# BuzzLord/godot-audio-spatializer

Measured on AMD Instinct MI355X. Metric: mixed AudioFrames/s, higher is better.
Workload: dtype f32

## Files before the change

### godot-audio-spatializer_amd/csrc/k_hrtf_multi.hip

```cpp
#define GAS_USE_NT 1
#ifndef GAS_MULTI_L2_PREFETCH
#define GAS_MULTI_L2_PREFETCH 0
#endif
#include "gas_hrtf_wave.h"

namespace {

constexpr int MW = 8;
constexpr int MAXB = GAS_HRTF_MULTI_MAX_BLOCKS;

template <int SQ>
struct MultiLds {
	static constexpr int SLICES_F2 = MW * LDS_F2_HALF;
	static constexpr int FD_F2 = MW * 2 * 512;
	static constexpr int TOTAL_F2 = SLICES_F2 + FD_F2;
	static constexpr int HL = (8 - SQ) * 64;
	static constexpr int LEFT_BYTES = 160 * 1024 - TOTAL_F2 * 8 - 1024 * 8 - 64;
	static constexpr int HIST_ROWS = LEFT_BYTES / (MW * HL * 4);
};

__device__ __forceinline__ void lds_wait_at_least(const uint32_t *flag, uint32_t want) {
	while (__atomic_load_n(flag, __ATOMIC_RELAXED) < want) {
		__builtin_amdgcn_s_sleep(1);
	}
	__builtin_amdgcn_fence(__ATOMIC_ACQUIRE, "workgroup");
}

template <int SQ, bool HIST_LDS>
__global__ __launch_bounds__(MW * 64, GAS_HRTF_WAVES_PER_SIMD) void k_hrtf_multi(gas_group_args g, gas_hrtf_blocks mb, const uint32_t *__restrict__ peak_bits, uint32_t peak_all, gas_dev_state st, gas_hrtf_table tab, const float2 *__restrict__ tw, float *__restrict__ partials) {
	constexpr int FQ = 2 * SQ;
	constexpr int HQ = 8 - SQ;
	constexpr int NQ = 8 + SQ;
	constexpr uint32_t F = FQ * 64;
	constexpr uint32_t HL = HQ * 64;
	__shared__ float2 lds_all[MultiLds<SQ>::TOTAL_F2];
	__shared__ float2 tw_lds[1024];
	__shared__ float hist_lds[HIST_LDS ? MW * MultiLds<SQ>::HIST_ROWS * HL : 4];
	__shared__ uint32_t arrived, consumed;
	const int lane = threadIdx.x & 63;
	const int wave = __builtin_amdgcn_readfirstlane(threadIdx.x >> 6);
	float2 *lds = lds_all + wave * LDS_F2_HALF;
	float *my_hist = hist_lds + (HIST_LDS ? wave * MultiLds<SQ>::HIST_ROWS * HL : 0);
	float2 *fd = lds_all + MultiLds<SQ>::SLICES_F2;
	const uint32_t K = mb.k;

	const float4 tw_in = reinterpret_cast<const float4 *>(tw)[threadIdx.x & 511];
	if (threadIdx.x == 0) {
		arrived = 0;
		consumed = 0;
	}
	uint32_t first, last;
	wave_range(g.n, blockIdx.x * MW + wave, gridDim.x * MW, first, last);
	const uint32_t cnt = last - first;
	const bool have = (uint32_t)lane < cnt;
	uint32_t my_slot = 0, my_row = 0, my_dir = 0, my_flag = 0;
	float my_g0 = 0.0f, my_g1 = 0.0f;
	if (have) {
		const uint32_t e = first + lane;
		my_slot = g.slots ? g.slots[e] : g.slot_base + e;
		my_row = g.rows ? g.rows[e] : e;
	}
	gas_audio_frame raw[FQ];
	float rawh[HQ];
	if (cnt > 0) {
		const uint32_t s0 = (uint32_t)__builtin_amdgcn_readlane((int)my_slot, 0), r0 = (uint32_t)__builtin_amdgcn_readlane((int)my_row, 0);
		load_history<HQ>(st.hrtf_hist + (size_t)s0 * HL, lane, rawh);
#pragma unroll
		for (int q = 0; q < FQ; q++) {
			raw[q] = (GAS_ABL & 8) ? gas_audio_frame{ (float)lane, (float)r0 } : nt_load_frame(mb.src[0] + (size_t)r0 * F + lane + 64 * q);
		}
	}
	auto block_params = [&](uint32_t b, float keep_g, uint32_t keep_d, float &g1, uint32_t &d) {
		const gas_params *fr = mb.fresh[b];
		g1 = keep_g;
		d = keep_d;
		if (have && (fr || b == 0)) {
			const gas_params *P = fr ? fr + my_row : st.params + my_slot;
			const float2 gd = *reinterpret_cast<const float2 *>(&P->hrtf_gain);
			const uint32_t dd = __float_as_uint(gd.y);
			g1 = gd.x;
			d = dd < tab.dirs ? dd : 0;
		}
	};
	if (have) {
		my_g0 = st.hrtf_prev_gain[my_slot];
		const uint32_t e = first + lane;
		my_flag = peak_all ? 1u : (peak_bits ? (peak_bits[e >> 5] >> (e & 31)) & 1u : 0u);
	}
	block_params(0, 0.0f, 0, my_g1, my_dir);
	if (threadIdx.x < 512) {
		reinterpret_cast<float4 *>(tw_lds)[threadIdx.x] = tw_in;
	}
	__syncthreads();
	float2 t1[8], t2[8];
#pragma unroll
	for (int k = 0; k < 8; k++) {
		t1[k] = tw_lds[k * 64 + lane];
		t2[k] = tw_lds[(8 + k) * 64 + lane];
	}
	const float lane_f = (float)lane;
#if GAS_MULTI_L2_PREFETCH
	uint32_t pf_word = 0;
#endif

	for (uint32_t b = 0; b < K; b++) {
		float *peaks_b = mb.peaks[b];
		float2 aYL[8], aYR[8], zp[8];
		float4 hs[8];
#pragma unroll
		for (int j = 0; j < 8; j++) {
			aYL[j] = make_float2(0.0f, 0.0f);
			aYR[j] = make_float2(0.0f, 0.0f);
			zp[j] = make_float2(0.0f, 0.0f);
		}
		float nx_g1 = my_g1;
		uint32_t nx_dir = my_dir;
		if (b + 1 < K) {
			block_params(b + 1, my_g1, my_dir, nx_g1, nx_dir);
		}
		bool have_prev = false;
		uint32_t prev_flag = 0, prev_row = 0;
		auto products = [&](bool more, uint32_t next_dir) {
			float2 yl[8], yr[8];
			if (have_prev) {
				finish_spectra(lane, hs);
#pragma unroll
				for (int j = 0; j < 8; j++) {
					cmac_fixed(aYL[j], zp[j], hs[j].x, hs[j].y);
					cmac_fixed(aYR[j], zp[j], hs[j].z, hs[j].w);
				}
				if (prev_flag) {
#pragma unroll
					for (int j = 0; j < 8; j++) {
						yl[j] = cmul_fixed(zp[j], hs[j].x, hs[j].y);
						yr[j] = cmul_fixed(zp[j], hs[j].z, hs[j].w);
					}
				}
			}
			if (more) {
				issue_spectra(tab.spec, next_dir, lane, hs);
			}
			if (have_prev && prev_flag) {
				fft512<true>(yl, t1, t2, lds, lane);
				fft512<true>(yr, t1, t2, lds, lane);
				float pkl = 0.0f, pkr = 0.0f;
#pragma unroll
				for (int t = 0; t < SQ; t++) {
					pkl = fmaxf(pkl, fmaxf(fabsf(yl[HQ + t].x), fabsf(yl[HQ + t].y)));
					pkr = fmaxf(pkr, fmaxf(fabsf(yr[HQ + t].x), fabsf(yr[HQ + t].y)));
				}
				pkl = wave_max(pkl);
				pkr = wave_max(pkr);
				if (lane == 0) {
					peaks_b[(size_t)prev_row * 2] = pkl;
					peaks_b[(size_t)prev_row * 2 + 1] = pkr;
				}
			}
		};

		for (uint32_t i = 0; i < cnt; i++) {
			const uint32_t slot = (uint32_t)__builtin_amdgcn_readlane((int)my_slot, (int)i);
			const uint32_t row = (uint32_t)__builtin_amdgcn_readlane((int)my_row, (int)i);
			const uint32_t dir = (uint32_t)__builtin_amdgcn_readlane((int)my_dir, (int)i);
			const float g0 = __int_as_float(__builtin_amdgcn_readlane(__float_as_int(my_g0), (int)i));
			const float g1 = __int_as_float(__builtin_amdgcn_readlane(__float_as_int(my_g1), (int)i));
			const uint32_t flag = (uint32_t)__builtin_amdgcn_readlane((int)my_flag, (int)i);
			float xq[NQ];
			if (HIST_LDS && b > 0) {
				load_history<HQ>(my_hist + (size_t)i * HL, lane, rawh);
			}
#pragma unroll
			for (int q = 0; q < HQ; q++) {
				xq[q] = rawh[q];
			}
			float lf = lane_f;
			asm volatile("" : "+v"(lf));
#pragma unroll
			for (int q = 0; q < FQ; q++) {
				const float mono = (raw[q].left + raw[q].right) * 0.5f;
				const float t = (lf + (float)(64 * q)) * (1.0f / (float)F);
				xq[HQ + q] = mono * (g1 * t + (1 - t) * g0);
			}
			if (!HIST_LDS || b + 1 == K) {
				store_history<HQ>(st.hrtf_hist + (size_t)slot * HL, lane, &xq[FQ]);
			} else {
				store_history<HQ>(my_hist + (size_t)i * HL, lane, &xq[FQ]);
			}
			const bool wrap = i + 1 == cnt;
			if (!wrap || b + 1 < K) {
				const uint32_t ni = wrap ? 0u : i + 1;
				const uint32_t nslot = (uint32_t)__builtin_amdgcn_readlane((int)my_slot, (int)ni);
				const uint32_t nrow = (uint32_t)__builtin_amdgcn_readlane((int)my_row, (int)ni);
				const gas_audio_frame *nsrc = mb.src[wrap ? b + 1 : b] + (size_t)nrow * F;
				if (!HIST_LDS || (b == 0 && !wrap)) {
					load_history<HQ>(st.hrtf_hist + (size_t)nslot * HL, lane, rawh);
				}
#pragma unroll
				for (int q = 0; q < FQ; q++) {
					raw[q] = (GAS_ABL & 8) ? gas_audio_frame{ (float)lane, (float)nrow } : nt_load_frame(nsrc + lane + 64 * q);
				}
			}
			float2 zs[8];
#pragma unroll
			for (int j = 0; j < 8; j++) {
				zs[j] = make_float2(xq[j], xq[j + SQ]);
			}
			fft512<false>(zs, t1, t2, lds, lane);
			products(true, dir);
#if GAS_MULTI_L2_PREFETCH
			{
				asm volatile("" ::"v"(pf_word));
				const uint32_t i2 = i + 2, over = i2 / cnt, ni2 = i2 - over * cnt;
				if (b + over < K) {
					const uint32_t row2 = (uint32_t)__builtin_amdgcn_readlane((int)my_row, (int)ni2);
					const char *p2 = reinterpret_cast<const char *>(mb.src[b + over] + (size_t)row2 * F);
					pf_word = *reinterpret_cast<const uint32_t *>(p2 + ((uint32_t)lane * 128u) % (F * 8u));
				}
			}
#endif
#pragma unroll
			for (int j = 0; j < 8; j++) {
				zp[j] = zs[j];
			}
			have_prev = true;
			prev_flag = flag;
			prev_row = row;
		}
		const int ep0 = (int)(2 * (b & 3));
		const gas_deferred_reduce job = mb.job[b];
		float4 jr[JOB_ROWS];
		const uint32_t jw = (uint32_t)((wave - ep0 - 2) & 7), jx = blockIdx.x & 7, ji = blockIdx.x >> 3;
		const uint32_t job_col = (((ji >> 1) * 8 + jx) * 8) + (ji & 1) * 4 + jw;
		const bool job_mine = job.partials != nullptr && jw < GAS_HRTF_JOB_WAVES && job_col < job.elems / 4;
		products(false, 0);

		lds_wait_at_least(&consumed, 2 * b);
#pragma unroll
		for (int j = 0; j < 8; j++) {
			fd[(wave * 2 + 0) * 512 + j * 64 + lane] = aYL[j];
			fd[(wave * 2 + 1) * 512 + j * 64 + lane] = aYR[j];
		}
		__builtin_amdgcn_fence(__ATOMIC_RELEASE, "workgroup");
		if (lane == 0) {
			__atomic_fetch_add(&arrived, 1u, __ATOMIC_RELAXED);
		}
		if (job_mine) {
			job_issue(job, job_col, lane, jr);
			job_finish(job, job_col, lane, jr);
		}
		if (wave == ep0 || wave == ep0 + 1) {
			const int ear = wave - ep0;
			lds_wait_at_least(&arrived, MW * (b + 1));
			float2 y[8];
#pragma unroll
			for (int j = 0; j < 8; j++) {
				y[j] = fd[ear * 512 + j * 64 + lane];
			}
#pragma unroll
			for (int w = 1; w < MW; w++) {
#pragma unroll
				for (int j = 0; j < 8; j++) {
					y[j] = cadd(y[j], fd[(w * 2 + ear) * 512 + j * 64 + lane]);
				}
			}
			__builtin_amdgcn_fence(__ATOMIC_RELEASE, "workgroup");
			if (lane == 0) {
				__atomic_fetch_add(&consumed, 1u, __ATOMIC_RELAXED);
			}
			fft512<true>(y, t1, t2, lds, lane);
			float *my_partial = partials + ((size_t)mb.p_offset[b] + blockIdx.x) * (size_t)(F * 2);
#pragma unroll
			for (int t = 0; t < SQ; t++) {
				const int fa = lane + 64 * t, fb = lane + 64 * (SQ + t);
				my_partial[fa * 2 + ear] = y[HQ + t].x;
				my_partial[fb * 2 + ear] = y[HQ + t].y;
			}
		}
		if (have && !my_flag) {
			*reinterpret_cast<float2 *>(peaks_b + (size_t)my_row * 2) = make_float2(__builtin_inff(), __builtin_inff());
		}
		my_g0 = my_g1;
		my_g1 = nx_g1;
		my_dir = nx_dir;
	}

	if (have) {
		st.hrtf_prev_gain[my_slot] = my_g0;
		if (mb.last_fresh) {
			const float4 *src4 = reinterpret_cast<const float4 *>(mb.last_fresh + my_row);
			float4 *dst4 = reinterpret_cast<float4 *>(st.params + my_slot);
#pragma unroll
			for (int k = 0; k < 8; k++) {
				dst4[k] = src4[k];
			}
		}
	}
}

}

bool gas_hrtf_multi_hist_in_lds(uint32_t n, uint32_t frames) {
	const uint32_t wgs = gas_hrtf_uni_partials(n);
	const uint32_t per_wave = (n + wgs * MW - 1) / (wgs * MW);
	switch (frames / 128) {
		case 1:
			return per_wave <= (uint32_t)MultiLds<1>::HIST_ROWS;
		case 2:
			return per_wave <= (uint32_t)MultiLds<2>::HIST_ROWS;
		case 3:
			return per_wave <= (uint32_t)MultiLds<3>::HIST_ROWS;
		default:
			return per_wave <= (uint32_t)MultiLds<4>::HIST_ROWS;
	}
}

hipError_t gas_launch_hrtf_multi(hipStream_t stream, const gas_group_args &g, const gas_hrtf_blocks &mb, const uint32_t *peak_bits, bool peak_all, const gas_dev_state &st, const gas_hrtf_table &tab, const float2 *twiddles, uint32_t frames, uint32_t hist_len, float *partials) {
	if (g.n == 0 || mb.k == 0) {
		return hipSuccess;
	}
	const uint32_t wgs = gas_hrtf_uni_partials(g.n);
	if (frames % 128 != 0 || frames > 512 || hist_len != 512 - frames / 2 || g.order != nullptr || mb.k > (uint32_t)MAXB || g.n < wgs * MW || g.n > wgs * MW * 64 || gas_hrtf_uni_waves() != (uint32_t)MW) {
		return hipErrorInvalidValue;
	}
	dim3 grid(wgs), block(MW * 64);
	const uint32_t all = peak_all ? 1u : 0u;
	const uint32_t per_wave = (g.n + wgs * MW - 1) / (wgs * MW);
#define GAS_MULTI_CASE(SQv)                                                                                                                     \
	case SQv:                                                                                                                                   \
		if (per_wave <= (uint32_t)MultiLds<SQv>::HIST_ROWS) {                                                                                   \
			hipLaunchKernelGGL((k_hrtf_multi<SQv, true>), grid, block, 0, stream, g, mb, peak_bits, all, st, tab, twiddles, partials);          \
		} else {                                                                                                                                \
			hipLaunchKernelGGL((k_hrtf_multi<SQv, false>), grid, block, 0, stream, g, mb, peak_bits, all, st, tab, twiddles, partials);         \
		}                                                                                                                                       \
		break;
	switch (frames / 128) {
		GAS_MULTI_CASE(1)
		GAS_MULTI_CASE(2)
		GAS_MULTI_CASE(3)
		GAS_MULTI_CASE(4)
		default:
			return hipErrorInvalidValue;
	}
#undef GAS_MULTI_CASE
	return hipGetLastError();
}
```

Baseline: 387.6 billion.

## Defer block epilogues into next block's loop and offload one flagged peak FFT to helper wave

The per-block epilogue (cross-wave reduction, inverse FFT, partial write) now runs inside the next block's products step, so it overlaps with other waves' work instead of stalling at the end of each block. The first wave with a flagged row hands that row's spectra through an LDS mailbox (reusing the twiddle buffer) to a designated helper wave, which computes the exact peak. The aim is to balance the FFT load across waves. It adds mailbox synchronisation counters, static_asserts on the role assignment, and a trailing epilogue after the block loop. Reusing tw_lds as the mailbox depends on twiddles already being held in registers.

```diff
diff --git a/godot-audio-spatializer_amd/csrc/k_hrtf_multi.hip b/godot-audio-spatializer_amd/csrc/k_hrtf_multi.hip
--- a/godot-audio-spatializer_amd/csrc/k_hrtf_multi.hip
+++ b/godot-audio-spatializer_amd/csrc/k_hrtf_multi.hip
@@ -18,6 +18,30 @@
 	static constexpr int LEFT_BYTES = 160 * 1024 - TOTAL_F2 * 8 - 1024 * 8 - 64;
 	static constexpr int HIST_ROWS = LEFT_BYTES / (MW * HL * 4);
 };
+
+constexpr int pe0(uint32_t b) {
+	return (int)(2 * (b & 3));
+}
+constexpr int helper(uint32_t b, int owner) {
+	const int odd = (int)((b >> 2) & 1);
+	const int h = (pe0(b) + 2 + odd) & 7;
+	return h != owner ? h : (pe0(b) + 2 + (odd ^ 1)) & 7;
+}
+constexpr bool helper_is_free(int what) {
+	for (uint32_t b = 0; b < 16; b++) {
+		for (int owner = -1; owner < 8; owner++) {
+			const int h = helper(b, owner);
+			const int jw = (h - pe0(b + 1) - 2) & 7;
+			if ((what == 0 && h == owner) || (what == 1 && (h == pe0(b) || h == pe0(b) + 1)) || (what == 2 && jw < GAS_HRTF_JOB_WAVES) || h < 0 || h >= MW) {
+				return false;
+			}
+		}
+	}
+	return true;
+}
+static_assert(helper_is_free(0), "the helper is never the owner (the owner's mailbox write waits for the helper's read)");
+static_assert(helper_is_free(1), "the helper of block b is not in the epilogue pair of block b (one duty per wave and block)");
+static_assert(helper_is_free(2), "the helper of block b is not a job wave of block b + 1");
 
 __device__ __forceinline__ void lds_wait_at_least(const uint32_t *flag, uint32_t want) {
 	while (__atomic_load_n(flag, __ATOMIC_RELAXED) < want) {
@@ -36,7 +60,7 @@
 	__shared__ float2 lds_all[MultiLds<SQ>::TOTAL_F2];
 	__shared__ float2 tw_lds[1024];
 	__shared__ float hist_lds[HIST_LDS ? MW * MultiLds<SQ>::HIST_ROWS * HL : 4];
-	__shared__ uint32_t arrived, consumed;
+	__shared__ uint32_t arrived, consumed, mail_read;
 	const int lane = threadIdx.x & 63;
 	const int wave = __builtin_amdgcn_readfirstlane(threadIdx.x >> 6);
 	float2 *lds = lds_all + wave * LDS_F2_HALF;
@@ -48,6 +72,7 @@
 	if (threadIdx.x == 0) {
 		arrived = 0;
 		consumed = 0;
+		mail_read = 0;
 	}
 	uint32_t first, last;
 	wave_range(g.n, blockIdx.x * MW + wave, gridDim.x * MW, first, last);
@@ -91,6 +116,13 @@
 	if (threadIdx.x < 512) {
 		reinterpret_cast<float4 *>(tw_lds)[threadIdx.x] = tw_in;
 	}
+	const uint64_t flagged = __ballot(my_flag != 0);
+	const uint32_t own_i = flagged ? (uint32_t)__builtin_ctzll(flagged) : 0u;
+	uint32_t *wave_flagged = reinterpret_cast<uint32_t *>(fd), *wave_row = wave_flagged + MW;
+	if (lane == 0) {
+		wave_flagged[wave] = flagged ? 1u : 0u;
+		wave_row[wave] = (uint32_t)__builtin_amdgcn_readlane((int)my_row, (int)own_i);
+	}
 	__syncthreads();
 	float2 t1[8], t2[8];
 #pragma unroll
@@ -98,13 +130,82 @@
 		t1[k] = tw_lds[k * 64 + lane];
 		t2[k] = tw_lds[(8 + k) * 64 + lane];
 	}
+	const uint64_t flagged_waves = __ballot(lane < MW && wave_flagged[lane & (MW - 1)] != 0);
+	const int owner = flagged_waves ? (int)__builtin_ctzll(flagged_waves) : -1;
+	const uint32_t owner_row = (uint32_t)__builtin_amdgcn_readfirstlane((int)wave_row[owner < 0 ? 0 : owner]);
+	const bool i_own = wave == owner;
+	__syncthreads();
+	float2 *mail = tw_lds;
 	const float lane_f = (float)lane;
 #if GAS_MULTI_L2_PREFETCH
 	uint32_t pf_word = 0;
 #endif
 
+	auto epilogue = [&](uint32_t eb, int ear) {
+		lds_wait_at_least(&arrived, MW * (eb + 1));
+		float2 y[8];
+#pragma unroll
+		for (int j = 0; j < 8; j++) {
+			y[j] = fd[ear * 512 + j * 64 + lane];
+		}
+#pragma nounroll
+		for (int w = 1; w < MW; w++) {
+#pragma unroll
+			for (int j = 0; j < 8; j++) {
+				y[j] = cadd(y[j], fd[(w * 2 + ear) * 512 + j * 64 + lane]);
+			}
+		}
+		__builtin_amdgcn_fence(__ATOMIC_RELEASE, "workgroup");
+		if (lane == 0) {
+			__atomic_fetch_add(&consumed, 1u, __ATOMIC_RELAXED);
+		}
+		fft512<true>(y, t1, t2, lds, lane);
+		float *my_partial = partials + ((size_t)mb.p_offset[eb] + blockIdx.x) * (size_t)(F * 2);
+#pragma unroll
+		for (int t = 0; t < SQ; t++) {
+			const int fa = lane + 64 * t, fb = lane + 64 * (SQ + t);
+			my_partial[fa * 2 + ear] = y[HQ + t].x;
+			my_partial[fb * 2 + ear] = y[HQ + t].y;
+		}
+	};
+	auto exact_peak = [&](float2 (&yl)[8], float2 (&yr)[8], float *peaks, uint32_t row) {
+		fft512<true>(yl, t1, t2, lds, lane);
+		fft512<true>(yr, t1, t2, lds, lane);
+		float pkl = 0.0f, pkr = 0.0f;
+#pragma unroll
+		for (int t = 0; t < SQ; t++) {
+			pkl = fmaxf(pkl, fmaxf(fabsf(yl[HQ + t].x), fabsf(yl[HQ + t].y)));
+			pkr = fmaxf(pkr, fmaxf(fabsf(yr[HQ + t].x), fabsf(yr[HQ + t].y)));
+		}
+		pkl = wave_max(pkl);
+		pkr = wave_max(pkr);
+		if (lane == 0) {
+			peaks[(size_t)row * 2] = pkl;
+			peaks[(size_t)row * 2 + 1] = pkr;
+		}
+	};
+	auto helper_duty = [&](uint32_t hb) {
+		lds_wait_at_least(&arrived, MW * (hb + 1));
+		float2 yl[8], yr[8];
+#pragma unroll
+		for (int j = 0; j < 8; j++) {
+			yl[j] = mail[j * 64 + lane];
+			yr[j] = mail[512 + j * 64 + lane];
+		}
+		__builtin_amdgcn_fence(__ATOMIC_RELEASE, "workgroup");
+		if (lane == 0) {
+			__atomic_fetch_add(&mail_read, 1u, __ATOMIC_RELAXED);
+		}
+		exact_peak(yl, yr, mb.peaks[hb], owner_row);
+	};
+
 	for (uint32_t b = 0; b < K; b++) {
 		float *peaks_b = mb.peaks[b];
+		uint32_t duty = 0;
+		if (b > 0) {
+			const int p = pe0(b - 1);
+			duty = (wave == p || wave == p + 1) ? 1u : ((owner >= 0 && wave == helper(b - 1, owner)) ? 2u : 0u);
+		}
 		float2 aYL[8], aYR[8], zp[8];
 		float4 hs[8];
 #pragma unroll
@@ -120,6 +221,7 @@
 		}
 		bool have_prev = false;
 		uint32_t prev_flag = 0, prev_row = 0;
+		bool prev_handed = false;
 		auto products = [&](bool more, uint32_t next_dir) {
 			float2 yl[8], yr[8];
 			if (have_prev) {
@@ -141,20 +243,24 @@
 				issue_spectra(tab.spec, next_dir, lane, hs);
 			}
 			if (have_prev && prev_flag) {
-				fft512<true>(yl, t1, t2, lds, lane);
-				fft512<true>(yr, t1, t2, lds, lane);
-				float pkl = 0.0f, pkr = 0.0f;
-#pragma unroll
-				for (int t = 0; t < SQ; t++) {
-					pkl = fmaxf(pkl, fmaxf(fabsf(yl[HQ + t].x), fabsf(yl[HQ + t].y)));
-					pkr = fmaxf(pkr, fmaxf(fabsf(yr[HQ + t].x), fabsf(yr[HQ + t].y)));
-				}
-				pkl = wave_max(pkl);
-				pkr = wave_max(pkr);
-				if (lane == 0) {
-					peaks_b[(size_t)prev_row * 2] = pkl;
-					peaks_b[(size_t)prev_row * 2 + 1] = pkr;
-				}
+				if (prev_handed) {
+					lds_wait_at_least(&mail_read, b);
+#pragma unroll
+					for (int j = 0; j < 8; j++) {
+						mail[j * 64 + lane] = yl[j];
+						mail[512 + j * 64 + lane] = yr[j];
+					}
+				} else {
+					exact_peak(yl, yr, peaks_b, prev_row);
+				}
+			}
+			if (have_prev && duty) {
+				if (duty == 1) {
+					epilogue(b - 1, wave - pe0(b - 1));
+				} else {
+					helper_duty(b - 1);
+				}
+				duty = 0;
 			}
 		};
 
@@ -225,8 +331,9 @@
 			have_prev = true;
 			prev_flag = flag;
 			prev_row = row;
-		}
-		const int ep0 = (int)(2 * (b & 3));
+			prev_handed = i_own && i == own_i;
+		}
+		const int ep0 = pe0(b);
 		const gas_deferred_reduce job = mb.job[b];
 		float4 jr[JOB_ROWS];
 		const uint32_t jw = (uint32_t)((wave - ep0 - 2) & 7), jx = blockIdx.x & 7, ji = blockIdx.x >> 3;
@@ -248,34 +355,6 @@
 			job_issue(job, job_col, lane, jr);
 			job_finish(job, job_col, lane, jr);
 		}
-		if (wave == ep0 || wave == ep0 + 1) {
-			const int ear = wave - ep0;
-			lds_wait_at_least(&arrived, MW * (b + 1));
-			float2 y[8];
-#pragma unroll
-			for (int j = 0; j < 8; j++) {
-				y[j] = fd[ear * 512 + j * 64 + lane];
-			}
-#pragma unroll
-			for (int w = 1; w < MW; w++) {
-#pragma unroll
-				for (int j = 0; j < 8; j++) {
-					y[j] = cadd(y[j], fd[(w * 2 + ear) * 512 + j * 64 + lane]);
-				}
-			}
-			__builtin_amdgcn_fence(__ATOMIC_RELEASE, "workgroup");
-			if (lane == 0) {
-				__atomic_fetch_add(&consumed, 1u, __ATOMIC_RELAXED);
-			}
-			fft512<true>(y, t1, t2, lds, lane);
-			float *my_partial = partials + ((size_t)mb.p_offset[b] + blockIdx.x) * (size_t)(F * 2);
-#pragma unroll
-			for (int t = 0; t < SQ; t++) {
-				const int fa = lane + 64 * t, fb = lane + 64 * (SQ + t);
-				my_partial[fa * 2 + ear] = y[HQ + t].x;
-				my_partial[fb * 2 + ear] = y[HQ + t].y;
-			}
-		}
 		if (have && !my_flag) {
 			*reinterpret_cast<float2 *>(peaks_b + (size_t)my_row * 2) = make_float2(__builtin_inff(), __builtin_inff());
 		}
@@ -284,6 +363,15 @@
 		my_dir = nx_dir;
 	}
 
+	{
+		const uint32_t lb = K - 1;
+		const int p = pe0(lb);
+		if (wave == p || wave == p + 1) {
+			epilogue(lb, wave - p);
+		} else if (owner >= 0 && wave == helper(lb, owner)) {
+			helper_duty(lb);
+		}
+	}
 	if (have) {
 		st.hrtf_prev_gain[my_slot] = my_g0;
 		if (mb.last_fresh) {
```

Result: no change. 387.4 billion (median of 2 runs) (-0.0%).
